# andr345/frtm-vos

Hardware: AMD Instinct MI355X
Metric: segmented frames/sec/GPU (480p, ResNet101, full CG iters) (higher is better)
Workload: dtype f32

## Files before the change

### frtm-vos_amd/csrc/cg_persistent.hip

```cpp
#include "resident_grid.h"

namespace {

using namespace resident;
constexpr int RMAX = 10;
constexpr int XR = RMAX + 4;
constexpr int SR = RMAX + 2;
constexpr int NMAX = FN;

struct Params {
  const float* X; const float* Bm; const float* cm; const float* sw;
  float* w2; float* vec; float* state; float* slabs; float* qbuf; unsigned* bar; unsigned* hbar;
  int N, c, h, w, R, parts, iters, has_p, apply_dff, fr, std_alpha, parity;
  float dff, lam2, invM, step;
  const int* guard; int guard_min; unsigned* stats;
  int count_run;
  long long spin_limit;
};

constexpr int L_VEC = 0;
constexpr int L_B = L_VEC + 7 * NMAX;
constexpr int L_C = L_B + 9 * RMAX * 64;
constexpr int L_S = L_C + RMAX * 64;
constexpr int L_T = L_S + SR * PW;
constexpr int L_RED = L_T + RMAX * PW;
constexpr int L_SRED = L_RED + NWAVE * SR * 64;
constexpr int L_FLAG = L_SRED + 32;
constexpr int L_TOTAL = L_FLAG + 4;

__global__ __launch_bounds__(NT) void k_cg_run_persistent(const Params P) {
  extern __shared__ __attribute__((aligned(16))) float lds[];
  float* vb = lds + L_VEC; float* vr = vb + NMAX; float* vrp = vr + NMAX; float* vp = vrp + NMAX; float* vq = vp + NMAX;
  float* vx = vq + NMAX; float* vw = vx + NMAX;
  float (*Bl)[RMAX][64] = (float (*)[RMAX][64])(lds + L_B);
  float (*cl)[64] = (float (*)[64])(lds + L_C);
  float (*sl)[PW] = (float (*)[PW])(lds + L_S);
  float (*tl)[PW] = (float (*)[PW])(lds + L_T);
  float (*red)[SR][64] = (float (*)[SR][64])(lds + L_RED);
  float* gl = vq;
  float* sred = lds + L_SRED;
  int* sh_flag_p = (int*)(lds + L_FLAG);

  const int tid = threadIdx.x, lane = tid & 63, wid = tid >> 6;
  const int G = gridDim.x, g = blockIdx.x;
  if (P.guard != nullptr && *P.guard < P.guard_min) {
    if (g == 0 && tid == 0 && P.stats && P.count_run) atomicAdd(P.stats + 1, 1u);
    return;
  }
  const int n_s = g / P.parts, part = g - n_s * P.parts;
  const int r0 = part * P.R;
  const int R = min(P.R, P.h - r0);
  const int c = P.c, h = P.h, w = P.w, n = c * 9;
  GridBarrier gb(P.bar, P.hbar, P.stats, P.spin_limit, sh_flag_p);
  const bool stamp_on = (g == 0) && (P.bar[3] != 0u);
  int n_stamp = 0;
  auto stamp = [&]() { if (stamp_on && tid == 0 && n_stamp < 250) { ((int*)P.qbuf)[NMAX + n_stamp] = (int)(wall_clock64() & 0x7fffffff); } ++n_stamp; };
  stamp();

  float xr[CPW][XR];
  load_rows<RMAX>(xr, P.X, (size_t)n_s * c, c, h, w, r0, P.R, lane, wid);
  load_maps<RMAX>(Bl, cl, sl, tl, P.Bm, P.cm, n_s, h, w, r0, R);
  for (int i = tid; i < NMAX; i += NT) {
    const bool on = i < n;
    vw[i] = on ? P.w2[i] : 0.f;
    vp[i] = (on && P.has_p) ? P.vec[3 * n + i] : 0.f;
    vrp[i] = (on && P.has_p) ? P.vec[2 * n + i] : 0.f;
    vb[i] = vr[i] = vq[i] = vx[i] = 0.f;
  }
  const float swn = P.sw[n_s];
  if (!gb.join()) return;
  stamp();

  auto apply = [&](const float* v, bool with_c) -> bool {
    partial_scores<RMAX>(xr, v, red, [&](int i, float s) {
      const int j = i >> 6, x = i & 63;
      const int yy = r0 - 1 + j;
      sl[j][x + 1] = (x < w && (unsigned)yy < (unsigned)h && j < R + 2) ? s : 0.f;
    });
    __syncthreads();
    stamp();
    stencil<RMAX>(Bl, cl, sl, tl, R, w, with_c, swn);
    stamp();
    weight_gradient<RMAX>(xr, tl, gl, P.slabs + (size_t)g * NMAX);
    stamp();
    if (!gb.sync()) return false;
    stamp();
    const int epw = (n + G - 1) / G;
    for (int e0 = wid; e0 < epw; e0 += NWAVE) {
      const int e = g * epw + e0;
      if (e < n) {
        float s = 0.f;
        for (int k = lane; k < G; k += 64) s += ld_l2(P.slabs + (size_t)k * NMAX + e);
        s = wave_sum_to63(s);
        if (lane == 63) st_wt(P.qbuf + e, s);
      }
    }
    stamp();
    if (!gb.sync()) return false;
    stamp();
    for (int i = tid; i < NMAX; i += NT) vq[i] = i < n ? ld_l2(P.qbuf + i) + P.lam2 * v[i] : 0.f;
    __syncthreads();
    stamp();
    return true;
  };

  if (!apply(vw, true)) return;
  float rho_cur;
  {
    float d0 = 0.f, d1 = 0.f;
    for (int i = tid; i < NMAX; i += NT) {
      const float bv = -vq[i];
      vb[i] = bv; vr[i] = bv;
      const float z = bv * P.invM;
      d0 += bv * z;
      if (P.has_p && !P.fr) d1 += vrp[i] * z;
    }
    bsum2(d0, d1, sred);
    float beta = 0.f;
    if (P.has_p) {
      float rho1 = P.state[0];
      if (P.apply_dff) rho1 = rho1 / P.dff;
      const float vv = P.fr ? d0 / rho1 : (d0 - d1) / rho1;
      beta = (vv < 0.f) ? 0.f : vv;
    }
    for (int i = tid; i < NMAX; i += NT) {
      const float z = vr[i] * P.invM;
      vp[i] = P.has_p ? (z + vp[i] * beta) : z;
    }
    rho_cur = d0;
    __syncthreads();
  }
  float alpha = 0.f, beta_last = 0.f, rho_prev = P.state[0];
  for (int it = 0; it < P.iters; ++it) {
    if (!apply(vp, false)) return;
    const bool first = it == 0, last = it == P.iters - 1;
    float pq = 0.f, pr = 0.f;
    for (int i = tid; i < NMAX; i += NT) { pq += vp[i] * vq[i]; pr += vp[i] * vr[i]; }
    bsum2(pq, pr, sred);
    alpha = P.std_alpha ? rho_cur / pq : pr / pq;
    float rn_ = 0.f, r2_ = 0.f;
    for (int i = tid; i < NMAX; i += NT) {
      const float rv = vr[i], pv = vp[i];
// ... 96 lines not shown
```

### frtm-vos_amd/csrc/joint_persistent.hip

```cpp
#include "resident_grid.h"

namespace {

using namespace resident;
constexpr int GCH = CPW * NWAVE;
constexpr int RMAX = 8;
constexpr int XR = RMAX + 4;
constexpr int SR = RMAX + 2;

struct JParams {
  const float* X; const float* Z; const float* Bm; const float* cm; const float* sw;
  const float* w1T;
  float* w1;
  float* w2;
  float* vec; float* state;
  float* spart; float* slabs; float* Fbuf; float* dots;
  unsigned* bar; unsigned* hbar; unsigned* stats;
  int N, Cin, c, h, w, R, parts, NGr, cpo, own_stride, iters, has_p, apply_dff, fr, std_alpha;
  float dff, lam1, lam2, invM1, invM2, step;
  long long spin_limit;
};

constexpr int L_W2 = 0;
constexpr int L_F = L_W2 + FN;
constexpr int L_FZ = L_F + FN;
constexpr int L_GL = L_FZ + FN;
constexpr int L_GX = L_GL + FN;
constexpr int L_B = L_GX + FN;
constexpr int L_C = L_B + 9 * RMAX * 64;
constexpr int L_S = L_C + RMAX * 64;
constexpr int L_T = L_S + SR * PW;
constexpr int L_RED = L_T + RMAX * PW;
constexpr int L_SRED = L_RED + NWAVE * SR * 64;
constexpr int L_FLAG = L_SRED + 32;
constexpr int L_FIXED = L_FLAG + 4;

__global__ __launch_bounds__(NT) void k_joint_run_persistent(const JParams P) {
  extern __shared__ __attribute__((aligned(16))) float lds[];
  float* w2l = lds + L_W2; float* vF = lds + L_F; float* vFz = lds + L_FZ; float* gl = lds + L_GL; float* gx = lds + L_GX;
  float (*Bl)[RMAX][64] = (float (*)[RMAX][64])(lds + L_B);
  float (*cl)[64] = (float (*)[64])(lds + L_C);
  float (*sl)[PW] = (float (*)[PW])(lds + L_S);
  float (*tl)[PW] = (float (*)[PW])(lds + L_T);
  float (*red)[SR][64] = (float (*)[SR][64])(lds + L_RED);
  float* sred = lds + L_SRED;
  int* sh_flag_p = (int*)(lds + L_FLAG);
  const int OS = P.own_stride;
  float* vb = lds + L_FIXED; float* vr = vb + OS; float* vrp = vr + OS; float* vp = vrp + OS; float* vq = vp + OS; float* vx = vq + OS;
  float* vw = vx + OS;

  const int tid = threadIdx.x, lane = tid & 63, wid = tid >> 6;
  const int G = gridDim.x, bid = blockIdx.x;
  const int KK = P.N * P.parts, NG = P.NGr + 1;
  const int g = bid / KK, k = bid - g * KK;
  const int n_s = k / P.parts, part = k - n_s * P.parts;
  const int r0 = part * P.R;
  const int R = min(P.R, P.h - r0);
  const int c = P.c, h = P.h, w = P.w, Cin = P.Cin;
  const bool zgrp = g == P.NGr;
  const int gbase = zgrp ? 0 : g * GCH;
  const int gcnt = zgrp ? c : min(GCH, Cin - gbase);
  const int n1 = Cin * c;
  const int o0 = min(k * P.cpo, gcnt), o1 = min((k + 1) * P.cpo, gcnt), ocnt = o1 - o0;
  const int per = zgrp ? 9 : c;
  const int own = ocnt * per;
  const int vbase = zgrp ? n1 + o0 * 9 : (gbase + o0) * c;
  const float lam = zgrp ? P.lam2 : P.lam1, invM = zgrp ? P.invM2 : P.invM1;
  GridBarrier gb(P.bar, P.hbar, P.stats, P.spin_limit, sh_flag_p);

  float xr[CPW][XR];
  load_rows<RMAX>(xr, zgrp ? P.Z : P.X, zgrp ? (size_t)n_s * c : (size_t)n_s * Cin + gbase, gcnt, h, w, r0, P.R, lane, wid);
  load_maps<RMAX>(Bl, cl, sl, tl, P.Bm, P.cm, n_s, h, w, r0, R);
  for (int i = tid; i < FN; i += NT) { w2l[i] = i < c * 9 ? P.w2[i] : 0.f; vF[i] = 0.f; vFz[i] = 0.f; gx[i] = 0.f; }
  for (int i = tid; i < OS; i += NT) {
    const bool on = i < own;
    vw[i] = on ? (zgrp ? P.w2[o0 * 9 + i] : P.w1T[(size_t)(gbase + o0) * c + i]) : 0.f;
    vp[i] = (on && P.has_p) ? P.vec[(size_t)3 * (n1 + c * 9) + vbase + i] : 0.f;
    vrp[i] = (on && P.has_p) ? P.vec[(size_t)2 * (n1 + c * 9) + vbase + i] : 0.f;
    vb[i] = vr[i] = vq[i] = vx[i] = 0.f;
  }
  const float swn = P.sw[n_s];
  if (!gb.join()) return;

  auto publish_compose = [&](const float* v, int slot) {
    float* dst = P.Fbuf + ((size_t)slot * NG + g) * FN + o0 * 9;
    for (int e = tid; e < ocnt * 9; e += NT) {
      float s = 0.f;
      if (zgrp) s = v[e];
      else {
        const int chl = e / 9, tap = e - chl * 9;
        const float* vrow = v + chl * c;
        for (int cc = 0; cc < c; ++cc) s += vrow[cc] * w2l[cc * 9 + tap];
      }
      st_wt(dst + e, s);
    }
  };
  auto read_F = [&](float* dstl, int slot) {
    const float* src = P.Fbuf + ((size_t)slot * NG + g) * FN;
    for (int i = tid; i < FN; i += NT) dstl[i] = i < gcnt * 9 ? ld_l2(src + i) : 0.f;
  };
  auto publish_dots = [&](float a, float b, int slot) {
    if (tid == 0) { st_wt(P.dots + ((size_t)slot * G + bid) * 2, a); st_wt(P.dots + ((size_t)slot * G + bid) * 2 + 1, b); }
  };
  auto sum_dots = [&](float& a, float& b, int slot) {
    float sa = 0.f, sb = 0.f;
    if (wid == 0) {
      for (int q = lane; q < G; q += 64) { sa += ld_l2(P.dots + ((size_t)slot * G + q) * 2); sb += ld_l2(P.dots + ((size_t)slot * G + q) * 2 + 1); }
      sa = wave_sum_to63(sa); sb = wave_sum_to63(sb);
      if (lane == 63) { sred[0] = sa; sred[1] = sb; }
    }
    __syncthreads();
    a = sred[0]; b = sred[1];
    __syncthreads();
  };

  auto apply = [&](const float* v_own, bool with_c, bool scores_on) -> bool {
    float* sp = P.spart + ((size_t)k * NG + g) * (SR * 64);
    if (scores_on) {
      partial_scores<RMAX>(xr, vF, red, [&](int i, float s) { st_wt(sp + i, s); });
    } else {
      for (int i = tid; i < SR * 64; i += NT) st_wt(sp + i, 0.f);
    }
    if (!gb.sync()) return false;
    for (int i = tid; i < SR * 64; i += NT) {
      const int jj = i >> 6, x = i & 63;
      const int yy = r0 - 1 + jj;
      float s = 0.f;
      const float* base = P.spart + (size_t)k * NG * (SR * 64) + i;
      for (int q = 0; q < NG; ++q) s += ld_l2(base + (size_t)q * (SR * 64));
      sl[jj][x + 1] = (x < w && (unsigned)yy < (unsigned)h && jj < R + 2) ? s : 0.f;
    }
    __syncthreads();
    stencil<RMAX>(Bl, cl, sl, tl, R, w, with_c, swn);
    weight_gradient<RMAX>(xr, tl, gl, P.slabs + ((size_t)g * KK + k) * FN);
    if (!gb.sync()) return false;
    for (int e0 = wid; e0 < ocnt * 9; e0 += NWAVE) {
      const int e = o0 * 9 + e0;
      float s = 0.f;
      for (int q = lane; q < KK; q += 64) s += ld_l2(P.slabs + ((size_t)g * KK + q) * FN + e);
      s = wave_sum_to63(s);
      if (lane == 63) gx[e0] = s;
    }
    __syncthreads();
    for (int i = tid; i < OS; i += NT) {
      float qv = 0.f;
      if (i < own) {
        if (zgrp) qv = gx[i];
        else {
          const int chl = i / c, cc = i - chl * c;
          const float* gr = gx + chl * 9;
          const float* wr = w2l + cc * 9;
#pragma unroll
          for (int tap = 0; tap < 9; ++tap) qv += gr[tap] * wr[tap];
        }
        qv += lam * v_own[i];
      }
      vq[i] = qv;
    }
    __syncthreads();
    return true;
  };

  if (zgrp) { for (int i = tid; i < FN; i += NT) vF[i] = w2l[i]; }
  if (P.has_p) publish_compose(vp, 1);
  __syncthreads();
  if (!apply(vw, true, zgrp)) return;
  float rho_cur;
  {
    float d0 = 0.f, d1 = 0.f;
    for (int i = tid; i < OS; i += NT) {
      const float bv = -vq[i];
      vb[i] = bv; vr[i] = bv;
      const float z = bv * invM;
      d0 += bv * z;
      if (P.has_p && !P.fr) d1 += vrp[i] * z;
      vx[i] = z;
    }
    bsum2(d0, d1, sred);
    publish_dots(d0, d1, 0);
    publish_compose(vx, 0);
    if (!gb.sync()) return;
    sum_dots(d0, d1, 0);
    float beta = 0.f;
    if (P.has_p) {
      float rho1 = P.state[0];
      if (P.apply_dff) rho1 = rho1 / P.dff;
      const float vv = P.fr ? d0 / rho1 : (d0 - d1) / rho1;
      beta = (vv < 0.f) ? 0.f : vv;
    }
    read_F(vFz, 0);
    if (P.has_p) read_F(vF, 1);
    __syncthreads();
    for (int i = tid; i < FN; i += NT) vF[i] = P.has_p ? vFz[i] + vF[i] * beta : vFz[i];
    for (int i = tid; i < OS; i += NT) {
      const float z = vr[i] * invM;
      vp[i] = P.has_p ? (z + vp[i] * beta) : z;
      vx[i] = 0.f;
    }
    rho_cur = d0;
    __syncthreads();
  }
  float alpha = 0.f, beta_last = 0.f, rho_prev = P.state[0];
  for (int it = 0; it < P.iters; ++it) {
    if (!apply(vp, false, true)) return;
    const bool first = it == 0, last = it == P.iters - 1;
    float pq = 0.f, pr = 0.f;
    for (int i = tid; i < OS; i += NT) { pq += vp[i] * vq[i]; pr += vp[i] * vr[i]; }
    bsum2(pq, pr, sred);
    publish_dots(pq, pr, 1);
    if (!gb.sync()) return;
    sum_dots(pq, pr, 1);
    alpha = P.std_alpha ? rho_cur / pq : pr / pq;
    float rn_ = 0.f, r2_ = 0.f;
    for (int i = tid; i < OS; i += NT) {
      const float rv = vr[i], pv = vp[i];
      vrp[i] = rv;
      vx[i] = first ? pv * alpha : vx[i] + pv * alpha;
      float rn = rv;
      if (!last) { rn = rv - vq[i] * alpha; vr[i] = rn; }
      const float z = rn * invM;
      rn_ += rn * z;
      r2_ += rv * z;
    }
    rho_prev = rho_cur;
    if (!last) {
      for (int i = tid; i < OS; i += NT) vq[i] = vr[i] * invM;
      bsum2(rn_, r2_, sred);
      publish_dots(rn_, r2_, 0);
      publish_compose(vq, 0);
      if (!gb.sync()) return;
      sum_dots(rn_, r2_, 0);
      const float vv = P.fr ? rn_ / rho_cur : (rn_ - r2_) / rho_cur;
      beta_last = (vv < 0.f) ? 0.f : vv;
      read_F(vFz, 0);
      __syncthreads();
      for (int i = tid; i < FN; i += NT) vF[i] = vFz[i] + vF[i] * beta_last;
      for (int i = tid; i < OS; i += NT) vp[i] = vq[i] + vp[i] * beta_last;
      rho_cur = rn_;
    }
    __syncthreads();
  }
  if (!gb.sync()) return;
  if (tid == 0) {
    unsigned st;
    if (bid == 0) st = claim_commit(gb.abort_flag(), P.stats);
    else {
      const long long t0 = wall_clock64();
      while ((st = __hip_atomic_load(gb.abort_flag(), __ATOMIC_RELAXED, __HIP_MEMORY_SCOPE_AGENT)) == 0u) {
        __builtin_amdgcn_s_sleep(1);
        if (wall_clock64() - t0 > P.spin_limit) { st = give_up_or_committed(gb.abort_flag(), P.stats) ? 2u : 1u; break; }
      }
    }
    sh_flag_p[0] = st == 2u ? 1 : 0;
  }
  __syncthreads();
  if (!sh_flag_p[0]) return;
  const size_t n = (size_t)n1 + c * 9;
  for (int i = tid; i < own; i += NT) {
    P.vec[0 * n + vbase + i] = vb[i];
    P.vec[1 * n + vbase + i] = vr[i];
    P.vec[2 * n + vbase + i] = vrp[i];
    P.vec[3 * n + vbase + i] = vp[i];
    P.vec[4 * n + vbase + i] = vq[i];
    P.vec[5 * n + vbase + i] = vx[i];
    const float nv = vw[i] + P.step * vx[i];
    if (zgrp) P.w2[o0 * 9 + i] = nv;
    else { const int chl = i / c, cc = i - chl * c; P.w1[(size_t)cc * Cin + gbase + o0 + chl] = nv; }
  }
  if (bid == 0 && tid == 0) {
    P.state[0] = P.iters > 0 ? rho_prev : P.state[0];
    P.state[4] = rho_cur;
    P.state[1] = alpha;
    P.state[2] = beta_last;
  }
}

}

extern "C" {

int frtm_joint_persistent_plan(int N, int Cin, int c, int h, int w, int* out4) {
  if (N < 1 || Cin < 1 || c < 1 || c > GCH || w < 1 || w > 64 || h < 1) return 0;
  const int budget = resident_budget();
  const int NG = ceil_div(Cin, GCH) + 1;
  const int min_parts = ceil_div(h, RMAX);
  if ((long)NG * N * min_parts > budget) return 0;
  int parts = budget / (NG * N);
// ... 54 lines not shown
```

### frtm-vos_amd/csrc/resident_grid.h

```cpp
#pragma once
#include "frtm_common.h"
#include "../../include/frtm_hip.h"

namespace resident {

constexpr int NT = 512;
constexpr int NWAVE = 8;
constexpr int CPW = 12;
constexpr int PW = 66;
constexpr int FN = CPW * NWAVE * 9;

__device__ __forceinline__ void st_wt(float* p, float v) { __hip_atomic_store(p, v, __ATOMIC_RELAXED, __HIP_MEMORY_SCOPE_AGENT); }
__device__ __forceinline__ float ld_l2(const float* p) { return __hip_atomic_load(p, __ATOMIC_RELAXED, __HIP_MEMORY_SCOPE_AGENT); }

__device__ __forceinline__ bool give_up_or_committed(unsigned* abort_flag, unsigned* stats) {
  unsigned expected = 0u;
  const bool won = __hip_atomic_compare_exchange_strong(abort_flag, &expected, 1u, __ATOMIC_RELAXED, __ATOMIC_RELAXED, __HIP_MEMORY_SCOPE_AGENT);
  if (won && stats) __hip_atomic_fetch_add(stats + 2, 1u, __ATOMIC_RELAXED, __HIP_MEMORY_SCOPE_AGENT);
  return !won && expected == 2u;
}
__device__ __forceinline__ unsigned claim_commit(unsigned* abort_flag, unsigned* stats) {
  unsigned expected = 0u;
  const bool won = __hip_atomic_compare_exchange_strong(abort_flag, &expected, 2u, __ATOMIC_RELAXED, __ATOMIC_RELAXED, __HIP_MEMORY_SCOPE_AGENT);
  if (won && stats) __hip_atomic_fetch_add(stats + 3, 1u, __ATOMIC_RELAXED, __HIP_MEMORY_SCOPE_AGENT);
  return won ? 2u : expected;
}

__device__ __forceinline__ bool grid_sync(unsigned* counter, unsigned* abort_flag, unsigned* stats, unsigned target, long long limit, int* sh_flag) {
  asm volatile("s_waitcnt vmcnt(0)" ::: "memory");
  __syncthreads();
  if (threadIdx.x == 0) {
    __hip_atomic_fetch_add(counter, 1u, __ATOMIC_RELAXED, __HIP_MEMORY_SCOPE_AGENT);
    const long long t0 = wall_clock64();
    int ok = 1;
    while (__hip_atomic_load(counter, __ATOMIC_RELAXED, __HIP_MEMORY_SCOPE_AGENT) < target) {
      __builtin_amdgcn_s_sleep(2);
      if (__hip_atomic_load(abort_flag, __ATOMIC_RELAXED, __HIP_MEMORY_SCOPE_AGENT) == 1u) { ok = 0; break; }
      if (wall_clock64() - t0 > limit) { ok = give_up_or_committed(abort_flag, stats) ? 1 : 0; break; }
    }
    *sh_flag = ok;
  }
  __syncthreads();
  return *sh_flag != 0;
}

constexpr int HB_ARR = 0, HB_GEN = 128, HB_TOP = 256, HB_POP = 272, HB_WORDS = 288;
static_assert(HB_WORDS == FRTM_HBAR_WORDS, "the callers allocate FRTM_HBAR_WORDS words of hbar");
__device__ __forceinline__ bool hier_sync(unsigned* hbar, unsigned* abort_flag, unsigned* stats, int xcc, unsigned n_x, unsigned n_active,
                                          unsigned epoch, long long limit, int* sh_flag) {
  asm volatile("s_waitcnt vmcnt(0)" ::: "memory");
  __syncthreads();
  if (threadIdx.x == 0) {
    int ok = 1;
    const long long t0 = wall_clock64();
    const unsigned old = __hip_atomic_fetch_add(hbar + HB_ARR + 16 * xcc, 1u, __ATOMIC_RELAXED, __HIP_MEMORY_SCOPE_AGENT);
    if (old + 1u == epoch * n_x) {
      __hip_atomic_fetch_add(hbar + HB_TOP, 1u, __ATOMIC_RELAXED, __HIP_MEMORY_SCOPE_AGENT);
      while (__hip_atomic_load(hbar + HB_TOP, __ATOMIC_RELAXED, __HIP_MEMORY_SCOPE_AGENT) < epoch * n_active) {
        __builtin_amdgcn_s_sleep(1);
        if (__hip_atomic_load(abort_flag, __ATOMIC_RELAXED, __HIP_MEMORY_SCOPE_AGENT) == 1u) { ok = 0; break; }
        if (wall_clock64() - t0 > limit) { ok = give_up_or_committed(abort_flag, stats) ? 1 : 0; break; }
      }
      if (ok) __hip_atomic_store(hbar + HB_GEN + 16 * xcc, epoch, __ATOMIC_RELAXED, __HIP_MEMORY_SCOPE_AGENT);
    } else {
      while (__hip_atomic_load(hbar + HB_GEN + 16 * xcc, __ATOMIC_RELAXED, __HIP_MEMORY_SCOPE_AGENT) < epoch) {
        __builtin_amdgcn_s_sleep(1);
        if (__hip_atomic_load(abort_flag, __ATOMIC_RELAXED, __HIP_MEMORY_SCOPE_AGENT) == 1u) { ok = 0; break; }
        if (wall_clock64() - t0 > limit) { ok = give_up_or_committed(abort_flag, stats) ? 1 : 0; break; }
      }
    }
    *sh_flag = ok;
  }
  __syncthreads();
  return *sh_flag != 0;
}

struct GridBarrier {
  unsigned* bar; unsigned* hbar; unsigned* stats; long long limit; int* sh;
  int xcc = 0; unsigned n_x = 1, n_active = 1, epoch = 0, hepoch = 0;

  __device__ __forceinline__ GridBarrier(unsigned* bar_, unsigned* hbar_, unsigned* stats_, long long limit_, int* sh_)
      : bar(bar_), hbar(hbar_), stats(stats_), limit(limit_), sh(sh_) {}
  __device__ __forceinline__ unsigned* abort_flag() const { return bar + 2; }
  __device__ __forceinline__ bool flat_sync() { return grid_sync(bar, abort_flag(), stats, (++epoch) * gridDim.x, limit, sh); }
  __device__ __forceinline__ bool join() {
    if (threadIdx.x == 0) sh[0] = 1;
    if (hbar != nullptr) {
      if (threadIdx.x == 0) {
        const int x = (int)(__builtin_amdgcn_s_getreg((3 << 11) | 20) & 7u);
        sh[1] = x;
        __hip_atomic_fetch_add(hbar + HB_POP + x, 1u, __ATOMIC_RELAXED, __HIP_MEMORY_SCOPE_AGENT);
      }
      __syncthreads();
      if (!flat_sync()) return false;
      if (threadIdx.x == 0) {
        unsigned act = 0, mine = 0;
        for (int x = 0; x < 8; ++x) {
          const unsigned c_ = __hip_atomic_load(hbar + HB_POP + x, __ATOMIC_RELAXED, __HIP_MEMORY_SCOPE_AGENT);
          act += c_ > 0u ? 1u : 0u;
          if (x == sh[1]) mine = c_;
        }
        sh[2] = (int)mine; sh[3] = (int)act;
      }
      __syncthreads();
      xcc = sh[1]; n_x = (unsigned)sh[2]; n_active = (unsigned)sh[3];
    }
    __syncthreads();
    return true;
  }
  __device__ __forceinline__ bool sync() {
    if (hbar != nullptr) return hier_sync(hbar, abort_flag(), stats, xcc, n_x, n_active, ++hepoch, limit, sh);
    return flat_sync();
  }
};

template <int CTRL, int ROW_MASK>
__device__ __forceinline__ float dpp_add(float v) {
  const int moved = __builtin_amdgcn_update_dpp(0, __float_as_int(v), CTRL, ROW_MASK, 0xf, true);
  return v + __int_as_float(moved);
}
__device__ __forceinline__ float wave_sum_to63(float v) {
  v = dpp_add<0x111, 0xf>(v);
  v = dpp_add<0x112, 0xf>(v);
  v = dpp_add<0x114, 0xf>(v);
  v = dpp_add<0x118, 0xf>(v);
  v = dpp_add<0x142, 0xa>(v);
  v = dpp_add<0x143, 0xc>(v);
  return v;
}

template <int NW = NWAVE>
__device__ __forceinline__ void bsum2(float& a, float& b, float* red) {
  a = wave_sum_to63(a);
  b = wave_sum_to63(b);
  const int lane = threadIdx.x & 63, wid = threadIdx.x >> 6;
  __syncthreads();
  if (lane == 63) { red[wid] = a; red[16 + wid] = b; }
  __syncthreads();
  float ta = 0.f, tb = 0.f;
#pragma unroll
  for (int i = 0; i < NW; ++i) { ta += red[i]; tb += red[16 + i]; }
  a = ta; b = tb;
}


template <int RMAX>
__device__ __forceinline__ void load_rows(float (&xr)[CPW][RMAX + 4], const float* X, size_t first, const int& cnt, const int& h, const int& w,
                                          const int& r0, const int& PR, const int& lane, const int& wid) {
  const int hw = h * w;
#pragma unroll
  for (int k = 0; k < CPW; ++k) {
    const int ch = wid * CPW + k;
    const float* Xc = X + (first + min(ch, cnt - 1)) * hw;
#pragma unroll
    for (int i = 0; i < RMAX + 4; ++i) {
      const int yy = r0 - 2 + i;
      const bool ok = ch < cnt && lane < w && (unsigned)yy < (unsigned)h && i < PR + 4;
      xr[k][i] = ok ? Xc[yy * w + lane] : 0.f;
    }
  }
}

template <int RMAX>
__device__ __forceinline__ void load_maps(float (*Bl)[RMAX][64], float (*cl)[64], float (*sl)[PW], float (*tl)[PW], const float* Bm, const float* cm,
                                          int n_s, int h, int w, int r0, int R) {
  const int tid = threadIdx.x, hw = h * w;
  for (int i = tid; i < 9 * RMAX * 64; i += NT) {
    const int d = i / (RMAX * 64), rr = (i / 64) % RMAX, x = i & 63;
    (&Bl[0][0][0])[i] = (rr < R && x < w) ? Bm[((size_t)n_s * 9 + d) * hw + (r0 + rr) * w + x] : 0.f;
  }
  for (int i = tid; i < RMAX * 64; i += NT) {
    const int rr = i / 64, x = i & 63;
    (&cl[0][0])[i] = (rr < R && x < w) ? cm[(size_t)n_s * hw + (r0 + rr) * w + x] : 0.f;
  }
  for (int i = tid; i < (RMAX + 2) * PW; i += NT) (&sl[0][0])[i] = 0.f;
  for (int i = tid; i < RMAX * PW; i += NT) (&tl[0][0])[i] = 0.f;
}

template <int RMAX, class Sink>
__device__ __forceinline__ void partial_scores(const float (&xr)[CPW][RMAX + 4], const float* f_all, float (*red)[RMAX + 2][64], Sink sink) {
  constexpr int SR = RMAX + 2;
  const int tid = threadIdx.x, lane = tid & 63, wid = tid >> 6;
  float S0[SR], S1[SR], S2[SR];
#pragma unroll
  for (int j = 0; j < SR; ++j) { S0[j] = 0.f; S1[j] = 0.f; S2[j] = 0.f; }
#pragma unroll
  for (int k = 0; k < CPW; ++k) {
    const float* f = f_all + (wid * CPW + k) * 9;
#pragma unroll
    for (int dy = 0; dy < 3; ++dy) {
      const float f0 = f[dy * 3 + 0], f1 = f[dy * 3 + 1], f2_ = f[dy * 3 + 2];
#pragma unroll
      for (int j = 0; j < SR; ++j) {
        const float xv = xr[k][j + dy];
        S0[j] += f0 * xv; S1[j] += f1 * xv; S2[j] += f2_ * xv;
      }
    }
  }
#pragma unroll
  for (int j = 0; j < SR; ++j) {
    const float l = __shfl_up(S0[j], 1, 64), r = __shfl_down(S2[j], 1, 64);
    red[wid][j][lane] = (lane > 0 ? l : 0.f) + S1[j] + (lane < 63 ? r : 0.f);
  }
  __syncthreads();
  for (int i = tid; i < SR * 64; i += NT) {
    const int j = i >> 6, x = i & 63;
    float s = 0.f;
#pragma unroll
    for (int q = 0; q < NWAVE; q += 4) s += (red[q][j][x] + red[q + 1][j][x]) + (red[q + 2][j][x] + red[q + 3][j][x]);
    sink(i, s);
  }
}

template <int RMAX>
__device__ __forceinline__ void stencil(float (*Bl)[RMAX][64], float (*cl)[64], float (*sl)[PW], float (*tl)[PW], int R, int w, bool with_c, float swn) {
  const int lane = threadIdx.x & 63, wid = threadIdx.x >> 6;
  for (int rr = wid; rr < RMAX; rr += NWAVE) {
    float acc = 0.f;
    if (rr < R && lane < w) {
#pragma unroll
      for (int dy = 0; dy < 3; ++dy)
#pragma unroll
        for (int dx = 0; dx < 3; ++dx) acc += Bl[dy * 3 + dx][rr][lane] * sl[rr + dy][lane + dx];
      if (with_c) acc -= cl[rr][lane];
      acc *= swn;
    }
    tl[rr][lane + 1] = acc;
  }
  __syncthreads();
}

template <int RMAX>
__device__ __forceinline__ void weight_gradient(const float (&xr)[CPW][RMAX + 4], float (*tl)[PW], float* gl, float* slab) {
  const int tid = threadIdx.x, lane = tid & 63, wid = tid >> 6;
  float tv[RMAX][3];
#pragma unroll
  for (int rr = 0; rr < RMAX; ++rr)
#pragma unroll
    for (int dx = 0; dx < 3; ++dx) tv[rr][dx] = tl[rr][lane + 2 - dx];
#pragma unroll
  for (int k = 0; k < CPW; ++k) {
    float a[9];
#pragma unroll
    for (int e = 0; e < 9; ++e) a[e] = 0.f;
#pragma unroll
    for (int rr = 0; rr < RMAX; ++rr)
#pragma unroll
      for (int dy = 0; dy < 3; ++dy) {
        const float xv = xr[k][rr + dy + 1];
#pragma unroll
        for (int dx = 0; dx < 3; ++dx) a[dy * 3 + dx] += tv[rr][dx] * xv;
      }
    float* dst = gl + (wid * CPW + k) * 9;
#pragma unroll
    for (int e = 0; e < 9; ++e) {
      const float tot = wave_sum_to63(a[e]);
      if (lane == 63) dst[e] = tot;
    }
  }
  __syncthreads();
  for (int i = tid; i < FN; i += NT) st_wt(slab + i, gl[i]);
}


static inline int resident_budget() {
  static int cached[16] = {0};
  int dev = 0;
  if (hipGetDevice(&dev) != hipSuccess || dev < 0 || dev >= 16) { (void)hipGetLastError(); return 240; }
  if (cached[dev] == 0) {
    int cus = 0;
    if (hipDeviceGetAttribute(&cus, hipDeviceAttributeMultiprocessorCount, dev) != hipSuccess || cus <= 0) { (void)hipGetLastError(); cus = 256; }
    cached[dev] = cus - cus / 16;
  }
  return cached[dev];
}

static inline long long resident_spin_limit(int debug_abort) { return debug_abort ? 0LL : 400000LL; }

static inline int resident_reset_words(unsigned* bar, unsigned* hbar, hipStream_t stream) {
  FRTM_HIP(hipMemsetAsync(bar, 0, 3 * sizeof(unsigned), stream));
  if (hbar) FRTM_HIP(hipMemsetAsync(hbar, 0, HB_WORDS * sizeof(unsigned), stream));
  return FRTM_OK;
}

}
```

### frtm-vos_amd/model/optimizer.py

```python
import torch

from .. import _hip as H
from ..lib.tensorlist import TensorList

HBAR_WORDS = 288


class MinimizationProblem:

    def __call__(self, x: TensorList) -> TensorList:
        raise NotImplementedError

    def ip_input(self, a, b):
        return sum(a.view(-1) @ b.view(-1))

    def initialize(self):
        pass

    def M1(self, x):
        return x


class GaussNewtonCG:

    debug_abort = False

    def __init__(self, problem: MinimizationProblem, variable: TensorList, cg_eps=0.0, fletcher_reeves=True,
                 standard_alpha=True, direction_forget_factor=0, step_alpha=1.0):
        self._generic = not all(hasattr(problem, need) for need in ('vector_layout', 'linearize', 'apply_A', 'apply_step'))
        self._g = dict(p=None, rho=torch.ones(1), r_prev=None)
        self.fletcher_reeves = fletcher_reeves
        self.standard_alpha = standard_alpha
        self.direction_forget_factor = direction_forget_factor
        self.problem = problem
        self.x = variable
        self.cg_eps = cg_eps
        self.step_alpha = step_alpha
        self._step_alpha0 = step_alpha
        self.residuals = torch.zeros(0)
        self.external_losses = []
        self.internal_losses = []
        self.gradient_mags = torch.zeros(0)
        self._n = None
        self._has_p = False
        self._buf = None
        self._pbuf = None
        self._jbuf = None
        self._guard = None
        self._last_of_run = True
        self._persistent_launched = False
        self._joint_launched = False
        self._gstats = None
        self._launched = []
        self._committed_seen = 0
        self._shadow = None
        self._aborts_handled = 0

    def _alloc(self):
        n1, n2, m1, m2 = self.problem.vector_layout()
        n = n1 + n2
        if self._buf is not None and self._n == n:
            return
        dev = self.x[0].device
        self._n, self._n1, self._n2 = n, n1, n2
        self._all = torch.zeros(6 * n + 8, device=dev)
        self._buf = self._all[:6 * n].view(6, n)
        self._state = self._all[6 * n:]
        self._state[:1].fill_(1.0)
        self._shadow = None
        self._partial = torch.zeros(4 * 64, device=dev)
        self._has_p = False
        self._stats()
        pr = self.problem
        if getattr(pr, 'joint', False) and hasattr(pr, 'persistent_joint_args'):
            self._joint_exchange(int(pr.mem.capacity), int(pr.Cin), int(pr.c), int(pr.h), int(pr.w))
        elif hasattr(pr, 'persistent_args'):
            self._filter_exchange()

    def _filter_exchange(self):
        if self._pbuf is None:
            dev = self._buf.device
            self._pbuf = (torch.empty(256 * 864, device=dev), torch.zeros(864 + 256, device=dev), torch.zeros(4, dtype=torch.int32, device=dev),
                          torch.zeros(HBAR_WORDS, dtype=torch.int32, device=dev))
        return self._pbuf

    def _joint_exchange(self, N, Cin, c, h, w):
        need = int(H.lib().frtm_joint_persistent_scratch(N, Cin, c, h, w))
        if need > 0 and (self._jbuf is None or self._jbuf[0].numel() < need):
# ... 323 lines not shown
```

### include/frtm_hip.h

```cpp
#ifndef FRTM_HIP_H
#define FRTM_HIP_H

#ifdef __cplusplus
extern "C" {
#endif

typedef void* frtm_stream_t;
typedef struct frtm_backbone frtm_backbone_t;

const char* frtm_last_error(void);
int frtm_version(void);
int frtm_device_info(int* out4_host);


#define FRTM_PX_PARTS 32
int frtm_pixel_weights(const void* y, int y_is_u8, int n, int H, int W, float tf,
                       float* out, float* scratch, frtm_stream_t stream);

int frtm_normal_build(const void* labels, int labels_is_u8, const float* pw, int n, int H, int W, int h, int w,
                      float tf, const int* slot_dev, int slot_host, float* Bmem, float* cmem,
                      float* scratch, const int* px_count_dev, frtm_stream_t stream);

int frtm_memory_update_window(float* sw, int cap, float lr, int num_samp_is_zero, int* state, const int* counts, int count_stride,
                              int min_count, int W, int* slots, const float* features, float* samples, int len, const float* labels,
                              size_t label_stride, int H, int Wd, int h, int w, float tf, float* Bmem, float* cmem, float* scratch,
                              frtm_stream_t stream);
int frtm_memory_next_slot(float* sw, int cap, float lr, int num_samp_is_zero, int* state,
                          const int* count_dev, int min_count, frtm_stream_t stream);

int frtm_memory_insert(const float* src, float* dst_base, int len, const int* slot_dev, frtm_stream_t stream);

int frtm_filter_scores(const float* X, const float* f, int N, int C, int h, int w,
                       float* out, int accumulate, frtm_stream_t stream);

int frtm_filter_scores_split(const float* X, const float* f, int N, int C, int h, int w, int splits, float* partial, frtm_stream_t stream);
int frtm_stencil_sum(const float* B, const float* c, const float* sw, const float* partials, int nsum, int N, int h, int w, float* t,
                     frtm_stream_t stream);
int frtm_stencil(const float* B, const float* c, const float* sw, const float* s, int N, int h, int w,
                 float* t, frtm_stream_t stream);

int frtm_filter_wgrad(const float* X, const float* t, int N, int C, int h, int w, int parts,
                      float* partial, frtm_stream_t stream);
int frtm_filter_wgrad_parts(int N, int C);
int frtm_filter_wgrad_parts_hw(int N, int C, int hw);

int frtm_filter_wgrad_stencil(const float* X, const float* s, const float* B, const float* c, const float* sw,
                              int N, int C, int h, int w, float* partial, frtm_stream_t stream);

int frtm_filter_igrad(const float* t, const float* f, int N, int C, int h, int w,
                      float* D, int pix_major, frtm_stream_t stream);

#define FRTM_CG_BLOCKS 64
int frtm_vec_reduce_slabs(const float* slabs, int nslab, int stride, int len, float lam2, const float* p,
                          float sign, float* q, frtm_stream_t stream);
int frtm_cg_begin(const float* b, float* r, const float* r_prev, int n1, int n2, float invM1, float invM2,
                  int has_p, float* partial, frtm_stream_t stream);
int frtm_cg_direction(const float* r, float* p, int n1, int n2, float invM1, float invM2, int has_p,
                      int apply_dff, int fletcher_reeves, float dff, float* state, const float* partial,
                      frtm_stream_t stream);
int frtm_cg_pq(const float* p, const float* q, const float* r, int n, float* partial, frtm_stream_t stream);
int frtm_cg_update(float* x, float* r, float* r_prev, const float* p, const float* q, int n1, int n2,
                   float invM1, float invM2, int first, int last, int standard_alpha, float* state,
                   float* partial, frtm_stream_t stream);
int frtm_filter_scores2(const float* X1, const float* f1, const float* X2, const float* f2, int N, int C, int h, int w, float* out,
                        frtm_stream_t stream);
int frtm_joint_mid(const float* s, const float* Bm, const float* cm, const float* sw, const float* Z, const float* w2, int N, int C,
                   int h, int w, int parts, float* partial, float* D, frtm_stream_t stream);
int frtm_joint_q_pq(const float* g1, int n1, float lam1, const float* slabs, int nslab, int stride, int n2, float lam2, const float* p1,
                    const float* p2, float sign, float* q, const float* r, float* partial, frtm_stream_t stream);
int frtm_joint_scores_composed(const float* X, const float* K, int Cx, const float* Z, const float* p2, int Cz, int N, int h, int w,
                               int splits, float* partial, frtm_stream_t stream);

int frtm_wide_parts(int h, int w);
int frtm_scores_wide(const float* X, const float* K, int Cx, const float* Z, const float* p2, int Cz, int N, int h, int w,
                     int splits, float* partial, frtm_stream_t stream);
int frtm_wgrad_wide(const float* X, const float* t, int N, int C, int h, int w, float* partial, frtm_stream_t stream);
int frtm_joint_q_pq_composed(const float* GX, int nslabX, int Cin, int c, const float* w2, float lam1, const float* slabs, int nslab,
                             int stride, int n2, float lam2, const float* p1, const float* p2, float sign, float* q, const float* r,
                             float* partial, frtm_stream_t stream);
int frtm_joint_compose(const float* p1, const float* w2, int Cin, int c, float* K, frtm_stream_t stream);
int frtm_joint_expand(const float* G, int nslab, const float* w2, int Cin, int c, float lam2, const float* p1, float sign, float* q1,
                      frtm_stream_t stream);

#define FRTM_HBAR_WORDS 288
int frtm_cg_persistent_plan(int N, int c, int h, int w, int* parts_out, int* rows_out);
int frtm_cg_run_persistent(const float* X, const float* Bm, const float* cm, const float* sw, int N, int c, int h, int w,
                           float* w2, float* vec, float* state, float* slabs, float* qbuf, unsigned* bar,
                           int iters, int has_p, int apply_dff, int fletcher_reeves, int standard_alpha, float dff,
                           float lam2, float invM, float step, frtm_stream_t stream);
int frtm_cg_run_persistent_guarded(const float* X, const float* Bm, const float* cm, const float* sw, int N, int c, int h, int w,
                                   float* w2, float* vec, float* state, float* slabs, float* qbuf, unsigned* bar,
                                   int iters, int has_p, int apply_dff, int fletcher_reeves, int standard_alpha, float dff,
                                   float lam2, float invM, float step, const int* guard_count, int guard_min, unsigned* stats,
                                   int count_run, int debug_abort, unsigned* hbar, frtm_stream_t stream);
int frtm_guarded_copy(float* dst, const float* src, int n, const int* guard_count, int guard_min, int mode, unsigned* stats, int count,
                      frtm_stream_t stream);
int frtm_cg_step_small(const float* slabs, int nslab, int stride, float lam2, float* x, float* r, float* r_prev,
                       float* p, float* q, int n, float invM, int first, int last, int standard_alpha,
                       int fletcher_reeves, float* state, frtm_stream_t stream);
int frtm_joint_persistent_plan(int N, int Cin, int c, int h, int w, int* out4);
size_t frtm_joint_persistent_scratch(int N, int Cin, int c, int h, int w);
int frtm_joint_run_persistent(const float* X, const float* Z, const float* Bm, const float* cm, const float* sw, int N, int Cin, int c, int h, int w,
                              const float* w1T, float* w1, float* w2, float* vec, float* state, float* scratch, unsigned* bar, unsigned* hbar,
                              int iters, int has_p, int apply_dff, int fletcher_reeves, int standard_alpha, float dff, float lam1, float lam2,
                              float invM1, float invM2, float step, unsigned* stats, int debug_abort, frtm_stream_t stream);
int frtm_vec_axpy(float* y, float a, const float* x, int n, frtm_stream_t stream);
int frtm_transpose2d(const float* in, int rows, int cols, float* out, frtm_stream_t stream);

typedef struct {
  int B, Cin, Hin, Win, Cout, ksize, stride, pad;
  int relu, out_transposed;
  int splitk;
  int tile;
  int w_layout;
  int ws_elems;
  int w_pitch;
} frtm_conv_desc;
#define FRTM_CONV_MAX_SPLITK 32
#define FRTM_WLAYOUT_GEMM 0
#define FRTM_WLAYOUT_HALO3X3 1
#define FRTM_WLAYOUT_WINO3X3 2
#define FRTM_CONV_WINO_ELEMS(Cout, Cin) ((((Cin) + 7) / 8 * 128) * (((Cout) + 31) / 32 * 32))
#define FRTM_WLAYOUT_WINO4 3
#define FRTM_CONV_WINO4_ELEMS(Cout, Cin) (36 * (((Cin) + 31) / 32 * 32) * (((Cout) + 31) / 32 * 32))
#define FRTM_CONV_WINO4_TILES(B, H, W) ((((B) * (((H) + 3) / 4) * (((W) + 3) / 4)) + 63) / 64 * 64)
#define FRTM_CONV_WINO4_WS_ELEMS(B, Cin, Cout, H, W) ((size_t)36 * ((Cin) + (Cout)) * FRTM_CONV_WINO4_TILES(B, H, W))
#define FRTM_WLAYOUT_WINO6 4
#define FRTM_CONV_WINO6_ELEMS(Cout, Cin) (64 * (((Cin) + 31) / 32 * 32) * (((Cout) + 31) / 32 * 32))
#define FRTM_CONV_WINO6_TILES(B, H, W) ((((B) * (((H) + 5) / 6) * (((W) + 5) / 6)) + 63) / 64 * 64)
#define FRTM_CONV_WINO6_WS_ELEMS(B, Cin, Cout, H, W) ((size_t)64 * ((Cin) + (Cout)) * FRTM_CONV_WINO6_TILES(B, H, W))
#define FRTM_WLAYOUT_BF16X3 5
#define FRTM_CONV_BF16X3_ELEMS(Cout, Cin) ((size_t)3 * (((Cin) + 15) / 16 * 16) * (((Cout) + 127) / 128 * 128) / 2)
#define FRTM_WLAYOUT_BF16X1 6
#define FRTM_CONV_BF16X1_ELEMS(Cout, Cin) ((size_t)(((Cin) + 15) / 16 * 16) * (((Cout) + 127) / 128 * 128) / 2)
#define FRTM_BF16X1_TILE_128x64 1
#define FRTM_BF16X1_TILE_64x64 2
#define FRTM_WINO_MIN_BLOCKS 512
#define FRTM_CONV_PACKED_ELEMS(Cout, Cin, k) \
  (((((Cin) * (k) * (k) + 31) / 32 * 32) > (((Cin) + 7) / 8 * 72) ? (((Cin) * (k) * (k) + 31) / 32 * 32) : (((Cin) + 7) / 8 * 72)) * (((Cout) + 31) / 32 * 32))
#define FRTM_TILE_64x64 1
#define FRTM_TILE_32x64 2
#define FRTM_TILE_128x64 3
#define FRTM_TILE_64x64_8W 4
#define FRTM_TILE_64x128_8W 7
#define FRTM_TILE_128x128_8W 8
#define FRTM_TILE_128x128_16W 9
#define FRTM_TILE_80x64 10
#define FRTM_TILE_G32_64x64 23
int frtm_conv_pack_weights(const float* w_oihw, int Cout, int Cin, int ksize, int layout,
                           float* wT, int* ktab, frtm_stream_t stream);
int frtm_conv2d(const frtm_conv_desc* desc_host, const float* in, const float* wT, const int* ktab,
                const float* scale, const float* shift, const float* residual, float* out,
                float* workspace, frtm_stream_t stream);

int frtm_backbone_create(int arch, frtm_backbone_t** out_host);
int frtm_backbone_destroy(frtm_backbone_t* bb);
int frtm_backbone_num_convs(const frtm_backbone_t* bb);
int frtm_backbone_conv_info(const frtm_backbone_t* bb, int idx, int* out6_host);
int frtm_backbone_set_conv_plan(frtm_backbone_t* bb, int idx, int tile, int splitk);
int frtm_backbone_set_conv(frtm_backbone_t* bb, int idx, const float* w_oihw, const float* bn_scale,
                           const float* bn_shift, frtm_stream_t stream);
int frtm_backbone_forward(frtm_backbone_t* bb, const unsigned char* image_u8, int B, int H, int W,
                          const float* norm_scale3, const float* norm_bias3,
                          float* layer1, float* layer2, float* layer3, float* layer4, float* layer5,
                          int stop_after_layer, frtm_stream_t stream);
int frtm_backbone_forward_at(frtm_backbone_t* bb, int lane_set, const unsigned char* image_u8, int B, int H, int W, const float* norm_scale3,
                             const float* norm_bias3, float* layer1, float* layer2, float* layer3, float* layer4, float* layer5,
// ... 120 lines not shown
```

Baseline: 653.3.

## Replace full grid barrier with per-tile group rendezvous and pack row registers as float2

In the joint persistent CG kernel, the barrier after publishing partial scores becomes a rendezvous among only the NG blocks sharing tile k. Each tile gets its own counter region in hbar, so blocks no longer wait for the whole grid. Input rows are also held as float2 vectors and the weight-gradient accumulation uses packed FMAs, aiming to cut VALU instruction count. The hbar allocation grows to hold the counters, and the monotonic per-apply targets depend on the counters being reset between runs.

```diff
diff --git a/frtm-vos_amd/csrc/cg_persistent.hip b/frtm-vos_amd/csrc/cg_persistent.hip
--- a/frtm-vos_amd/csrc/cg_persistent.hip
+++ b/frtm-vos_amd/csrc/cg_persistent.hip
@@ -57,7 +57,7 @@
   auto stamp = [&]() { if (stamp_on && tid == 0 && n_stamp < 250) { ((int*)P.qbuf)[NMAX + n_stamp] = (int)(wall_clock64() & 0x7fffffff); } ++n_stamp; };
   stamp();
 
-  float xr[CPW][XR];
+  f32x2 xr[CPW][XR / 2];
   load_rows<RMAX>(xr, P.X, (size_t)n_s * c, c, h, w, r0, P.R, lane, wid);
   load_maps<RMAX>(Bl, cl, sl, tl, P.Bm, P.cm, n_s, h, w, r0, R);
   for (int i = tid; i < NMAX; i += NT) {
diff --git a/frtm-vos_amd/csrc/joint_persistent.hip b/frtm-vos_amd/csrc/joint_persistent.hip
--- a/frtm-vos_amd/csrc/joint_persistent.hip
+++ b/frtm-vos_amd/csrc/joint_persistent.hip
@@ -68,7 +68,7 @@
   const float lam = zgrp ? P.lam2 : P.lam1, invM = zgrp ? P.invM2 : P.invM1;
   GridBarrier gb(P.bar, P.hbar, P.stats, P.spin_limit, sh_flag_p);
 
-  float xr[CPW][XR];
+  f32x2 xr[CPW][XR / 2];
   load_rows<RMAX>(xr, zgrp ? P.Z : P.X, zgrp ? (size_t)n_s * c : (size_t)n_s * Cin + gbase, gcnt, h, w, r0, P.R, lane, wid);
   load_maps<RMAX>(Bl, cl, sl, tl, P.Bm, P.cm, n_s, h, w, r0, R);
   for (int i = tid; i < FN; i += NT) { w2l[i] = i < c * 9 ? P.w2[i] : 0.f; vF[i] = 0.f; vFz[i] = 0.f; gx[i] = 0.f; }
@@ -114,14 +114,14 @@
     __syncthreads();
   };
 
-  auto apply = [&](const float* v_own, bool with_c, bool scores_on) -> bool {
+  auto apply = [&](const float* v_own, bool with_c, bool scores_on, int app) -> bool {
     float* sp = P.spart + ((size_t)k * NG + g) * (SR * 64);
     if (scores_on) {
       partial_scores<RMAX>(xr, vF, red, [&](int i, float s) { st_wt(sp + i, s); });
     } else {
       for (int i = tid; i < SR * 64; i += NT) st_wt(sp + i, 0.f);
     }
-    if (!gb.sync()) return false;
+    if (!gb.group_sync(k, KK, (unsigned)((app + 1) * NG))) return false;
     for (int i = tid; i < SR * 64; i += NT) {
       const int jj = i >> 6, x = i & 63;
       const int yy = r0 - 1 + jj;
@@ -164,7 +164,7 @@
   if (zgrp) { for (int i = tid; i < FN; i += NT) vF[i] = w2l[i]; }
   if (P.has_p) publish_compose(vp, 1);
   __syncthreads();
-  if (!apply(vw, true, zgrp)) return;
+  if (!apply(vw, true, zgrp, 0)) return;
   float rho_cur;
   {
     float d0 = 0.f, d1 = 0.f;
@@ -202,7 +202,7 @@
   }
   float alpha = 0.f, beta_last = 0.f, rho_prev = P.state[0];
   for (int it = 0; it < P.iters; ++it) {
-    if (!apply(vp, false, true)) return;
+    if (!apply(vp, false, true, it + 1)) return;
     const bool first = it == 0, last = it == P.iters - 1;
     float pq = 0.f, pr = 0.f;
     for (int i = tid; i < OS; i += NT) { pq += vp[i] * vq[i]; pr += vp[i] * vr[i]; }
diff --git a/frtm-vos_amd/csrc/resident_grid.h b/frtm-vos_amd/csrc/resident_grid.h
--- a/frtm-vos_amd/csrc/resident_grid.h
+++ b/frtm-vos_amd/csrc/resident_grid.h
@@ -44,7 +44,7 @@
   return *sh_flag != 0;
 }
 
-constexpr int HB_ARR = 0, HB_GEN = 128, HB_TOP = 256, HB_POP = 272, HB_WORDS = 288;
+constexpr int HB_ARR = 0, HB_GEN = 128, HB_TOP = 256, HB_POP = 272, HB_RDV = 288, RDV_MAX = 128, HB_WORDS = HB_RDV + 16 * RDV_MAX;
 static_assert(HB_WORDS == FRTM_HBAR_WORDS, "the callers allocate FRTM_HBAR_WORDS words of hbar");
 __device__ __forceinline__ bool hier_sync(unsigned* hbar, unsigned* abort_flag, unsigned* stats, int xcc, unsigned n_x, unsigned n_active,
                                           unsigned epoch, long long limit, int* sh_flag) {
@@ -112,6 +112,10 @@
     if (hbar != nullptr) return hier_sync(hbar, abort_flag(), stats, xcc, n_x, n_active, ++hepoch, limit, sh);
     return flat_sync();
   }
+  __device__ __forceinline__ bool group_sync(int k, int groups, unsigned target) {
+    if (hbar == nullptr || groups > RDV_MAX) return sync();
+    return grid_sync(hbar + HB_RDV + 16 * k, abort_flag(), stats, target, limit, sh);
+  }
 };
 
 template <int CTRL, int ROW_MASK>
@@ -143,9 +147,17 @@
   a = ta; b = tb;
 }
 
-
-template <int RMAX>
-__device__ __forceinline__ void load_rows(float (&xr)[CPW][RMAX + 4], const float* X, size_t first, const int& cnt, const int& h, const int& w,
+typedef float f32x2 __attribute__((ext_vector_type(2)));
+__device__ __forceinline__ f32x2 pk_fma(f32x2 a, float b, f32x2 c) { return __builtin_elementwise_fma(a, f32x2{b, b}, c); }
+template <int RMAX>
+__device__ __forceinline__ void pin_rows(f32x2 (&x)[(RMAX + 4) / 2]) {
+#pragma unroll
+  for (int i = 0; i < (RMAX + 4) / 2; ++i) asm volatile("" : "+v"(x[i]));
+}
+
+
+template <int RMAX>
+__device__ __forceinline__ void load_rows(f32x2 (&xr)[CPW][(RMAX + 4) / 2], const float* X, size_t first, const int& cnt, const int& h, const int& w,
                                           const int& r0, const int& PR, const int& lane, const int& wid) {
   const int hw = h * w;
 #pragma unroll
@@ -156,7 +168,7 @@
     for (int i = 0; i < RMAX + 4; ++i) {
       const int yy = r0 - 2 + i;
       const bool ok = ch < cnt && lane < w && (unsigned)yy < (unsigned)h && i < PR + 4;
-      xr[k][i] = ok ? Xc[yy * w + lane] : 0.f;
+      xr[k][i / 2][i & 1] = ok ? Xc[yy * w + lane] : 0.f;
     }
   }
 }
@@ -178,7 +190,7 @@
 }
 
 template <int RMAX, class Sink>
-__device__ __forceinline__ void partial_scores(const float (&xr)[CPW][RMAX + 4], const float* f_all, float (*red)[RMAX + 2][64], Sink sink) {
+__device__ __forceinline__ void partial_scores(f32x2 (&xr)[CPW][(RMAX + 4) / 2], const float* f_all, float (*red)[RMAX + 2][64], Sink sink) {
   constexpr int SR = RMAX + 2;
   const int tid = threadIdx.x, lane = tid & 63, wid = tid >> 6;
   float S0[SR], S1[SR], S2[SR];
@@ -187,12 +199,13 @@
 #pragma unroll
   for (int k = 0; k < CPW; ++k) {
     const float* f = f_all + (wid * CPW + k) * 9;
+    pin_rows<RMAX>(xr[k]);
 #pragma unroll
     for (int dy = 0; dy < 3; ++dy) {
       const float f0 = f[dy * 3 + 0], f1 = f[dy * 3 + 1], f2_ = f[dy * 3 + 2];
 #pragma unroll
       for (int j = 0; j < SR; ++j) {
-        const float xv = xr[k][j + dy];
+        const float xv = xr[k][(j + dy) / 2][(j + dy) & 1];
         S0[j] += f0 * xv; S1[j] += f1 * xv; S2[j] += f2_ * xv;
       }
     }
@@ -231,31 +244,33 @@
 }
 
 template <int RMAX>
-__device__ __forceinline__ void weight_gradient(const float (&xr)[CPW][RMAX + 4], float (*tl)[PW], float* gl, float* slab) {
+__device__ __forceinline__ void weight_gradient(f32x2 (&xr)[CPW][(RMAX + 4) / 2], float (*tl)[PW], float* gl, float* slab) {
   const int tid = threadIdx.x, lane = tid & 63, wid = tid >> 6;
-  float tv[RMAX][3];
-#pragma unroll
-  for (int rr = 0; rr < RMAX; ++rr)
-#pragma unroll
-    for (int dx = 0; dx < 3; ++dx) tv[rr][dx] = tl[rr][lane + 2 - dx];
+  f32x2 tv01[RMAX];
+  float tv2[RMAX];
+#pragma unroll
+  for (int rr = 0; rr < RMAX; ++rr) { tv01[rr] = f32x2{tl[rr][lane + 2], tl[rr][lane + 1]}; tv2[rr] = tl[rr][lane]; }
 #pragma unroll
   for (int k = 0; k < CPW; ++k) {
-    float a[9];
-#pragma unroll
-    for (int e = 0; e < 9; ++e) a[e] = 0.f;
+    f32x2 a01[3];
+    float a2[3];
+    pin_rows<RMAX>(xr[k]);
+#pragma unroll
+    for (int dy = 0; dy < 3; ++dy) { a01[dy] = f32x2{0.f, 0.f}; a2[dy] = 0.f; }
 #pragma unroll
     for (int rr = 0; rr < RMAX; ++rr)
 #pragma unroll
       for (int dy = 0; dy < 3; ++dy) {
-        const float xv = xr[k][rr + dy + 1];
-#pragma unroll
-        for (int dx = 0; dx < 3; ++dx) a[dy * 3 + dx] += tv[rr][dx] * xv;
+        const float xv = xr[k][(rr + dy + 1) / 2][(rr + dy + 1) & 1];
+        a01[dy] = pk_fma(tv01[rr], xv, a01[dy]); a2[dy] = __builtin_fmaf(tv2[rr], xv, a2[dy]);
       }
     float* dst = gl + (wid * CPW + k) * 9;
-#pragma unroll
-    for (int e = 0; e < 9; ++e) {
-      const float tot = wave_sum_to63(a[e]);
-      if (lane == 63) dst[e] = tot;
+    float tot[9];
+#pragma unroll
+    for (int e = 0; e < 9; ++e) tot[e] = wave_sum_to63(e % 3 == 0 ? a01[e / 3].x : e % 3 == 1 ? a01[e / 3].y : a2[e / 3]);
+    if (lane == 63) {
+#pragma unroll
+      for (int e = 0; e < 9; ++e) dst[e] = tot[e];
     }
   }
   __syncthreads();
diff --git a/frtm-vos_amd/model/optimizer.py b/frtm-vos_amd/model/optimizer.py
--- a/frtm-vos_amd/model/optimizer.py
+++ b/frtm-vos_amd/model/optimizer.py
@@ -3,7 +3,7 @@
 from .. import _hip as H
 from ..lib.tensorlist import TensorList
 
-HBAR_WORDS = 288
+HBAR_WORDS = 2336
 
 
 class MinimizationProblem:
diff --git a/include/frtm_hip.h b/include/frtm_hip.h
--- a/include/frtm_hip.h
+++ b/include/frtm_hip.h
@@ -82,7 +82,7 @@
 int frtm_joint_expand(const float* G, int nslab, const float* w2, int Cin, int c, float lam2, const float* p1, float sign, float* q1,
                       frtm_stream_t stream);
 
-#define FRTM_HBAR_WORDS 288
+#define FRTM_HBAR_WORDS 2336
 int frtm_cg_persistent_plan(int N, int c, int h, int w, int* parts_out, int* rows_out);
 int frtm_cg_run_persistent(const float* X, const float* Bm, const float* cm, const float* sw, int N, int c, int h, int w,
                            float* w2, float* vec, float* state, float* slabs, float* qbuf, unsigned* bar,
```

After: 655.6, median of 4. Within noise of the previous version (+0.4%).
